# G-U-N/Phased-Consistency-Model

Hardware: NVIDIA H100
Metric: distillation steps/sec (SD1.5 PCM-LoRA, bs=8/GPU) (higher is better)
Workload: dtype bf16

## Files before the change

pcm_b200/csrc/attn.cu:

```cuda
#include <stdio.h>
#include <stdlib.h>
#include "common.cuh"
#include "host_common.h"
#include "../../include/pcm_b200.h"

namespace pcm {

struct AttnParams {
  const bf16 *q, *k, *v, *o, *dout;
  bf16 *out, *dq, *dk, *dv;
  float *lse, *delta;
  int B, H, Sq, Skv, D;
  long long ldq, ldk, ldv, ldo;
  float scale;
};

__device__ __forceinline__ void cp_async16(void* smem_dst, const void* gsrc) {
  asm volatile("cp.async.cg.shared.global [%0], [%1], 16;" ::"r"(smem_u32(smem_dst)), "l"(gsrc)
               : "memory");
}
__device__ __forceinline__ void cp_async_commit() { asm volatile("cp.async.commit_group;" ::: "memory"); }
template <int N>
__device__ __forceinline__ void cp_async_wait() {
  asm volatile("cp.async.wait_group %0;" ::"n"(N) : "memory");
// ... 164 lines not shown
    if (row >= p.Sq) continue;
    const float inv = 1.f / l_run[r];
    bf16* orow = p.out + (static_cast<long long>(b) * p.Sq + row) * p.ldo + h * p.D;
#pragma unroll
    for (int i = 0; i < DP / 8; ++i) {
      const int col = i * 8 + (lane & 3) * 2;
      if (col < p.D)
        *reinterpret_cast<uint32_t*>(orow + col) =
            pack_bf16x2(oacc[i][2 * r] * inv, oacc[i][2 * r + 1] * inv);
    }
    if ((lane & 3) == 0 && p.lse)
      p.lse[(static_cast<long long>(b) * p.H + h) * p.Sq + row] = m_run[r] + log2f(l_run[r]);
  }
}

__global__ void attn_delta_kernel(const AttnParams p) {
  griddep_sync();
  const long long i = blockIdx.x * static_cast<long long>(blockDim.x) + threadIdx.x;
  const long long total = static_cast<long long>(p.B) * p.Sq * p.H;
  if (i >= total) return;
  const int h = static_cast<int>(i % p.H);
  const long long bs = i / p.H;
  const int s = static_cast<int>(bs % p.Sq);
  const int b = static_cast<int>(bs / p.Sq);
  const bf16* o = p.o + bs * p.ldo + h * p.D;
  const bf16* d = p.dout + bs * p.ldo + h * p.D;
  float acc = 0.f;
  for (int c = 0; c < p.D; c += 8) {
    const uint4 u = *reinterpret_cast<const uint4*>(o + c);
    const uint4 w = *reinterpret_cast<const uint4*>(d + c);
    const uint32_t uu[4] = {u.x, u.y, u.z, u.w}, ww[4] = {w.x, w.y, w.z, w.w};
#pragma unroll
    for (int k = 0; k < 4; ++k) {
      const float2 a = unpack_bf16x2(uu[k]), bb = unpack_bf16x2(ww[k]);
      acc += a.x * bb.x + a.y * bb.y;
    }
  }
  p.delta[(static_cast<long long>(b) * p.H + h) * p.Sq + s] = acc;
}

template <int DP>
__global__ void __launch_bounds__(128) attn_bwd_dkdv_kernel(const AttnParams p) {
  griddep_sync();
  constexpr int LDS = DP + 8, BQ = 64, BN = 64, T = 128;
  extern __shared__ __align__(16) uint8_t smem_attn[];
  bf16* sK = reinterpret_cast<bf16*>(smem_attn);
  bf16* sV = sK + BN * LDS;
  bf16* sQ = sV + BN * LDS;
  bf16* sdO = sQ + 2 * BQ * LDS;
  float* sL = reinterpret_cast<float*>(sdO + 2 * BQ * LDS);
  float* sD = sL + 2 * BQ;
  const int tid = threadIdx.x, warp = tid >> 5, lane = tid & 31;
  const int b = blockIdx.z, h = blockIdx.y, n0 = blockIdx.x * BN;
// ... 231 lines not shown
  static bool set = false;
  if (!set) {
    CUDA_TRY(cudaFuncSetAttribute(attn_fwd_kernel<DP>, cudaFuncAttributeMaxDynamicSharedMemorySize,
                                  static_cast<int>(smem)));
    set = true;
  }
  dim3 grid((p.Sq + 127) / 128, p.H, p.B);
  CUDA_TRY(launch_pdl(attn_fwd_kernel<DP>, dim3(grid), dim3(256), smem, stream, p));
  CUDA_TRY(cudaGetLastError());
  return 0;
}

template <int DP>
static int launch_bwd(const AttnParams& p, cudaStream_t stream) {
  constexpr int LDS = DP + 8;
  {
    const long long total = static_cast<long long>(p.B) * p.Sq * p.H;
    CUDA_TRY(launch_pdl(attn_delta_kernel, dim3(static_cast<int>((total + 127) / 128)), dim3(128), 0, stream, p));
  }
  const size_t smem1 = static_cast<size_t>(6 * 64) * LDS * sizeof(bf16) + 4 * 64 * sizeof(float);
  const size_t smem2 = static_cast<size_t>(6 * 64) * LDS * sizeof(bf16);
  static bool set = false;
  if (!set) {
    CUDA_TRY(cudaFuncSetAttribute(attn_bwd_dkdv_kernel<DP>,
                                  cudaFuncAttributeMaxDynamicSharedMemorySize,
                                  static_cast<int>(smem1)));
    CUDA_TRY(cudaFuncSetAttribute(attn_bwd_dq_kernel<DP>,
                                  cudaFuncAttributeMaxDynamicSharedMemorySize,
                                  static_cast<int>(smem2)));
    set = true;
  }
  CUDA_TRY(launch_pdl(attn_bwd_dkdv_kernel<DP>, dim3(dim3((p.Skv + 63) / 64, p.H, p.B)), dim3(128), smem1, stream, p));
  CUDA_TRY(launch_pdl(attn_bwd_dq_kernel<DP>, dim3(dim3((p.Sq + 63) / 64, p.H, p.B)), dim3(128), smem2, stream, p));
  CUDA_TRY(cudaGetLastError());
// ... 111 lines not shown
  AttnParams p{};
  p.q = reinterpret_cast<const bf16*>(q);
  p.k = reinterpret_cast<const bf16*>(k);
  p.v = reinterpret_cast<const bf16*>(v);
  p.o = reinterpret_cast<const bf16*>(o);
  p.dout = reinterpret_cast<const bf16*>(dout);
  p.lse = const_cast<float*>(lse);
  p.delta = delta;
  p.dq = reinterpret_cast<bf16*>(dq);
  p.dk = reinterpret_cast<bf16*>(dk);
  p.dv = reinterpret_cast<bf16*>(dv);
  p.B = B; p.H = H; p.Sq = Sq; p.Skv = Skv; p.D = D;
  p.ldq = ldq; p.ldk = ldk; p.ldv = ldv; p.ldo = ldo;
  p.scale = scale;
  cudaStream_t st = reinterpret_cast<cudaStream_t>(stream);
  if (D <= 64) {
    const long long total = static_cast<long long>(B) * Sq * H;
    CUDA_TRY(launch_pdl(attn_delta_kernel, dim3(static_cast<unsigned>((total + 127) / 128)), dim3(128), 0, st, p));
    const int rc = attn_bwd_wg(q, k, v, dout, lse, delta, dq, dk, dv, B, H, Sq, Skv, D, ldq, ldk, ldv, ldo, scale, st);
    if (rc <= 0) return rc;
  }
  DISPATCH_DP(D, launch_bwd);
}
```

pcm_b200/csrc/attn_wg.cu:

```cuda
#include <type_traits>

#include "common.cuh"
#include "wgmma.cuh"
#include "host_common.h"

namespace pcm {

namespace {

constexpr int kAwThreads = 384;
constexpr int kAwStages = 2;
constexpr int kBwdStages = 3;
constexpr int kTile = 64 * 128;

struct alignas(64) AttnWgParams {
  CUtensorMap q_map, k_map, v_map;
  bf16* out;
  float* lse;
  int H, Sq, Skv, D;
  long long ldo;
  float c;
};

__device__ __forceinline__ void keep_operand(uint32_t (&a)[4][4]) {
// ... 25 lines not shown
    mx[r] = fmaxf(mx[r], __shfl_xor_sync(0xffffffffu, mx[r], 2));
    const float mn = fmaxf(m_run[r], mx[r]);
    alpha[r] = exp2_ftz(m_run[r] - mn);
    m_run[r] = mn;
    rs[r] = 0.f;
  }
#pragma unroll
  for (int i = 0; i < 32; i += 2) {
    const int r = (i >> 1) & 1;
    const float p0 = exp2_ftz(__fsub_rn(s[i], m_run[r])), p1 = exp2_ftz(__fsub_rn(s[i + 1], m_run[r]));
    rs[r] += p0 + p1;
    pa[i >> 3][(i & 7) >> 1] = pack_bf16x2(p0, p1);
  }
}

template <int KB, int NV>
__global__ void __launch_bounds__(kAwThreads, 1) attn_fwd_wg_kernel(const __grid_constant__ AttnWgParams p) {
  static_assert(NV == 64 || (KB == 1 && NV == 40), "trimmed products only for one 64-column block");
  constexpr int KS = (NV + 15) / 16;
  extern __shared__ uint8_t smem_raw[];
  uint8_t* smem = reinterpret_cast<uint8_t*>((reinterpret_cast<uintptr_t>(smem_raw) + 1023) &
                                             ~static_cast<uintptr_t>(1023));
  uint8_t* sQ = smem;
  uint8_t* sK = sQ + 2 * KB * kTile;
  uint8_t* sV = sK + kAwStages * KB * kTile;
  __shared__ __align__(8) uint64_t q_bar;
  __shared__ __align__(8) uint64_t full_bar[kAwStages];
  __shared__ __align__(8) uint64_t empty_bar[kAwStages];

  const int wg = threadIdx.x >> 7;
  const int b = blockIdx.z, h = blockIdx.y, q0 = blockIdx.x * 128;
  const int nblk = (p.Skv + 63) / 64;
  constexpr uint32_t kv_bytes = 2 * KB * kTile;

// ... 33 lines not shown
  const int cw = wg - 1, et = threadIdx.x & 127, warp = et >> 5, lane = et & 31;
  uint8_t* myQ = sQ + cw * KB * kTile;
  mbar_wait(&q_bar, 0);
  if (p.D < KB * 64) {
    const int c0 = p.D >> 3, nch = KB * 8;
    for (int i = et; i < 64 * nch; i += 128) {
      const int row = i / nch, ch = i - row * nch;
      if (ch < c0) continue;
      const uint32_t a = smem_u32(myQ + (ch >> 3) * kTile) + row * 128 + (((ch & 7) ^ (row & 7)) << 4);
      sts128(a, 0u, 0u, 0u, 0u);
    }
    fence_proxy_async();
  }
  asm volatile("bar.sync %0, 128;" ::"r"(1 + cw) : "memory");

  float o[KB][NV / 2];
#pragma unroll
  for (int kb = 0; kb < KB; ++kb)
#pragma unroll
    for (int i = 0; i < NV / 2; ++i) o[kb][i] = 0.f;
  float m_run[2] = {-INFINITY, -INFINITY}, l_run[2] = {0.f, 0.f};
  const uint32_t q_addr = smem_u32(myQ);

  auto block = [&](int j, auto mask) {
    const int st = j % kAwStages;
    mbar_wait(&full_bar[st], (j / kAwStages) & 1);
    const uint32_t k_addr = smem_u32(sK + st * KB * kTile);
    const uint32_t v_addr = smem_u32(sV + st * KB * kTile);
    float s[32];
    wgmma_fence();
#pragma unroll
    for (int kb = 0; kb < KB; ++kb)
#pragma unroll
      for (int k = 0; k < KS; ++k)
        Wgmma<64, 0, 0>::mma(s, wgmma_desc_sw128(q_addr + kb * kTile + k * 32, 16, 1024),
                             wgmma_desc_sw128(k_addr + kb * kTile + k * 32, 16, 1024), (kb | k) != 0 ? 1u : 0u);
    wgmma_commit();
    wgmma_wait<0>();
    wgmma_fence_acc(s);

    float alpha[2], rs[2];
    uint32_t pa[4][4];
    fwd_softmax<decltype(mask)::value>(s, m_run, alpha, rs, pa, p.c, j * 64 + 2 * (lane & 3), p.Skv);
#pragma unroll
    for (int r = 0; r < 2; ++r) l_run[r] = __fmaf_rn(l_run[r], alpha[r], rs[r]);
    if (!__all_sync(0xffffffffu, alpha[0] == 1.f && alpha[1] == 1.f)) {
#pragma unroll
      for (int kb = 0; kb < KB; ++kb)
#pragma unroll
        for (int i = 0; i < NV / 2; ++i) o[kb][i] *= alpha[(i >> 1) & 1];
    }

    wgmma_fence();
#pragma unroll
    for (int kk = 0; kk < 4; ++kk)
#pragma unroll
      for (int kb = 0; kb < KB; ++kb)
        WgmmaRs<NV, 1>::mma(o[kb], pa[kk], wgmma_desc_sw128(v_addr + kb * kTile + kk * 2048, kTile, 1024), 1u);
    wgmma_commit();
    wgmma_wait<0>();
#pragma unroll
    for (int kb = 0; kb < KB; ++kb) wgmma_fence_acc(o[kb]);
    __syncwarp();
    if (et == 0) mbar_arrive(&empty_bar[st]);
  };
  const int nfull = p.Skv / 64;
  for (int j = 0; j < nfull; ++j) block(j, std::false_type());
  if (nfull < nblk) block(nfull, std::true_type());

#pragma unroll
  for (int r = 0; r < 2; ++r) {
    l_run[r] += __shfl_xor_sync(0xffffffffu, l_run[r], 1);
    l_run[r] += __shfl_xor_sync(0xffffffffu, l_run[r], 2);
  }
  const int row0 = q0 + 64 * cw + 16 * warp + (lane >> 2);
#pragma unroll
  for (int r = 0; r < 2; ++r) {
    const int row = row0 + 8 * r;
    if (row >= p.Sq) continue;
    const float inv = 1.f / l_run[r];
    bf16* orow = p.out + (static_cast<long long>(b) * p.Sq + row) * p.ldo + h * p.D;
#pragma unroll
    for (int kb = 0; kb < KB; ++kb)
#pragma unroll
      for (int q = 0; q < NV / 8; ++q) {
        const int col = kb * 64 + 8 * q + 2 * (lane & 3);
        if (col < p.D)
          *reinterpret_cast<uint32_t*>(orow + col) =
              pack_bf16x2(o[kb][4 * q + 2 * r] * inv, o[kb][4 * q + 2 * r + 1] * inv);
      }
    if ((lane & 3) == 0 && p.lse) p.lse[(static_cast<long long>(b) * p.H + h) * p.Sq + row] = m_run[r] + log2f(l_run[r]);
  }
}

struct alignas(64) AttnBwdParams {
  CUtensorMap fix0_map, fix1_map;
  CUtensorMap str0_map, str1_map;
  const float *lse, *delta;
  bf16 *out0, *out1;
  long long ld0, ld1;
  int H, Sq, Skv, D;
  int n_fix, n_str;
  float c, scale;
};

// ... 13 lines not shown
        l = lc[2 * (i >> 2) + e];
        d = dc[2 * (i >> 2) + e];
        ok = rvalid[r];
      } else {
        l = lrow[r];
        d = drow[r];
        ok = !MASK || kcol + 8 * (i >> 2) + e < Skv;
      }
      const float pv = ok ? exp2_ftz(__fmaf_rn(s[i + e], c, -l)) : 0.f;
      s[i + e] = pv;
      dp[i + e] = pv * (dp[i + e] - d);
    }
  }
}

template <bool KV, int NV>
__global__ void __launch_bounds__(kAwThreads, 1) attn_bwd_wg_kernel(const __grid_constant__ AttnBwdParams p) {
  constexpr int kStages = kBwdStages;
  constexpr int KS = (NV + 15) / 16;
  extern __shared__ uint8_t smem_raw[];
  uint8_t* smem = reinterpret_cast<uint8_t*>((reinterpret_cast<uintptr_t>(smem_raw) + 1023) &
                                             ~static_cast<uintptr_t>(1023));
  uint8_t* sF = smem;
  uint8_t* sS = sF + 4 * kTile;
  __shared__ __align__(8) uint64_t f_bar;
  __shared__ __align__(8) uint64_t full_bar[kStages];
  __shared__ __align__(8) uint64_t empty_bar[kStages];
  __shared__ float stats[2][2][2][64];

  const int wg = threadIdx.x >> 7;
  const int b = blockIdx.z, h = blockIdx.y, r0 = blockIdx.x * 128;
  const int nblk = (p.n_str + 63) / 64;
  const int col0 = h * p.D;

  if (threadIdx.x == 0) {
    tma_prefetch_desc(&p.fix0_map);
    tma_prefetch_desc(&p.fix1_map);
    tma_prefetch_desc(&p.str0_map);
    tma_prefetch_desc(&p.str1_map);
    mbar_init(&f_bar, 1);
    for (int i = 0; i < kStages; ++i) {
      mbar_init(&full_bar[i], 1);
      mbar_init(&empty_bar[i], 2);
    }
    fence_barrier_init();
  }
  __syncthreads();
  griddep_sync();

  if (wg == 0) {
    regs_dealloc<40>();
    if (threadIdx.x == 0) {
      mbar_arrive_expect_tx(&f_bar, 4 * kTile);
      for (int w = 0; w < 2; ++w) {
        tma_load_3d(sF + (2 * w) * kTile, &p.fix0_map, &f_bar, col0, r0 + 64 * w, b);
        tma_load_3d(sF + (2 * w + 1) * kTile, &p.fix1_map, &f_bar, col0, r0 + 64 * w, b);
      }
      for (int j = 0; j < nblk; ++j) {
        const int st = j % kStages;
        mbar_wait(&empty_bar[st], ((j / kStages) & 1) ^ 1);
        mbar_arrive_expect_tx(&full_bar[st], 2 * kTile);
        tma_load_3d(sS + (2 * st) * kTile, &p.str0_map, &full_bar[st], col0, j * 64, b);
        tma_load_3d(sS + (2 * st + 1) * kTile, &p.str1_map, &full_bar[st], col0, j * 64, b);
      }
    }
    return;
  }

  regs_alloc<232>();
  const int cw = wg - 1, et = threadIdx.x & 127, warp = et >> 5, lane = et & 31;
  uint8_t* myF = sF + 2 * cw * kTile;
  mbar_wait(&f_bar, 0);
  if (p.D < 64) {
    const int c0 = p.D >> 3;
    for (int i = et; i < 2 * 64 * 8; i += 128) {
      const int t = i >> 9, row = (i >> 3) & 63, ch = i & 7;
      if (ch < c0) continue;
      sts128(smem_u32(myF + t * kTile) + row * 128 + ((ch ^ (row & 7)) << 4), 0u, 0u, 0u, 0u);
    }
    fence_proxy_async();
  }
  asm volatile("bar.sync %0, 128;" ::"r"(1 + cw) : "memory");

  const float* L = p.lse + (static_cast<long long>(b) * p.H + h) * p.Sq;
  const float* Dl = p.delta + (static_cast<long long>(b) * p.H + h) * p.Sq;
  const int frow = r0 + 64 * cw + 16 * warp + (lane >> 2);
  float lrow[2] = {0.f, 0.f}, drow[2] = {0.f, 0.f};
  bool rvalid[2];
#pragma unroll
  for (int r = 0; r < 2; ++r) {
    rvalid[r] = frow + 8 * r < p.n_fix;
    if (!KV) {
      lrow[r] = rvalid[r] ? L[frow + 8 * r] : INFINITY;
      drow[r] = rvalid[r] ? Dl[frow + 8 * r] : 0.f;
    }
  }
  float acc0[NV / 2], acc1[NV / 2];
#pragma unroll
  for (int i = 0; i < NV / 2; ++i) acc0[i] = acc1[i] = 0.f;
  const uint32_t f0 = smem_u32(myF), f1 = f0 + kTile;
  const bool ragged = !KV && (p.Skv & 63) != 0;
  float s[32], dp[32];
  uint32_t pa[4][4], dsa[4][4];

  auto issue_sdp = [&](int st) {
    const uint32_t s0 = smem_u32(sS + 2 * st * kTile), s1 = s0 + kTile;
    Wgmma<64, 0, 0>::mma_first(s, wgmma_desc_sw128(f0, 16, 1024), wgmma_desc_sw128(s0, 16, 1024));
    Wgmma<64, 0, 0>::mma_first(dp, wgmma_desc_sw128(f1, 16, 1024), wgmma_desc_sw128(s1, 16, 1024));
#pragma unroll
    for (int k = 1; k < KS; ++k) {
      Wgmma<64, 0, 0>::mma(s, wgmma_desc_sw128(f0 + k * 32, 16, 1024), wgmma_desc_sw128(s0 + k * 32, 16, 1024), 1u);
      Wgmma<64, 0, 0>::mma(dp, wgmma_desc_sw128(f1 + k * 32, 16, 1024), wgmma_desc_sw128(s1 + k * 32, 16, 1024), 1u);
    }
    wgmma_commit();
  };
  auto issue_acc = [&](int st) {
    const uint32_t s0 = smem_u32(sS + 2 * st * kTile), s1 = s0 + kTile;
#pragma unroll
    for (int kk = 0; kk < 4; ++kk) {
      WgmmaRs<NV, 1>::mma(acc0, dsa[kk], wgmma_desc_sw128(s0 + kk * 2048, kTile, 1024), 1u);
      if (KV) WgmmaRs<NV, 1>::mma(acc1, pa[kk], wgmma_desc_sw128(s1 + kk * 2048, kTile, 1024), 1u);
    }
    wgmma_commit();
  };
  auto load_stat = [&](int j) {
    const int qi = j * 64 + (et & 63);
    if (et < 64) return qi < p.Sq ? L[qi] : INFINITY;
    return qi < p.Sq ? Dl[qi] : 0.f;
  };
  auto publish_stat = [&](int j, float v) {
    stats[cw][j & 1][et >> 6][et & 63] = v;
    asm volatile("bar.sync %0, 128;" ::"r"(1 + cw) : "memory");
  };
  auto elementwise = [&](int j) {
    const int kcol = j * 64 + 2 * (lane & 3);
    float lc[16], dc[16];
// ... 28 lines not shown
  pack_operand(dsa, dp);

  for (int j = 1; j < nblk; ++j) {
    const int st = j % kStages, pst = (j - 1) % kStages;
    mbar_wait(&full_bar[st], (j / kStages) & 1);
    wgmma_fence();
    issue_sdp(st);
    issue_acc(pst);
    if (KV) nxt = load_stat(j + 1);
    wgmma_wait<1>();
    wgmma_fence_acc(s);
    wgmma_fence_acc(dp);
    elementwise(j);
    if (KV) publish_stat(j + 1, nxt);
    wgmma_wait<0>();
    wgmma_fence_acc(acc0);
    wgmma_fence_acc(acc1);
    keep_operand(pa);
    keep_operand(dsa);
    __syncwarp();
    if (et == 0) mbar_arrive(&empty_bar[pst]);
    pack_operand(pa, s);
    pack_operand(dsa, dp);
  }
  wgmma_fence();
  issue_acc((nblk - 1) % kStages);
  wgmma_wait<0>();
  wgmma_fence_acc(acc0);
  wgmma_fence_acc(acc1);
  keep_operand(pa);
  keep_operand(dsa);

#pragma unroll
  for (int r = 0; r < 2; ++r) {
    if (!rvalid[r]) continue;
    const long long row = static_cast<long long>(b) * p.n_fix + frow + 8 * r;
    bf16* o0 = p.out0 + row * p.ld0 + col0;
    bf16* o1 = KV ? p.out1 + row * p.ld1 + col0 : nullptr;
#pragma unroll
    for (int q = 0; q < NV / 8; ++q) {
      const int col = 8 * q + 2 * (lane & 3);
      if (col < p.D) {
        *reinterpret_cast<uint32_t*>(o0 + col) =
            pack_bf16x2(acc0[4 * q + 2 * r] * p.scale, acc0[4 * q + 2 * r + 1] * p.scale);
        if (KV) *reinterpret_cast<uint32_t*>(o1 + col) = pack_bf16x2(acc1[4 * q + 2 * r], acc1[4 * q + 2 * r + 1]);
      }
    }
  }
}

int encode_seq_map(CUtensorMap* m, const void* base, int HD, int S, int B, long long ld) {
  if ((reinterpret_cast<uintptr_t>(base) & 15) != 0 || (ld & 7) != 0)
    return set_error("attention: tensor map base not 16-byte aligned or row stride not a multiple of 8");
  cuuint64_t dims[3] = {static_cast<cuuint64_t>(HD), static_cast<cuuint64_t>(S), static_cast<cuuint64_t>(B)};
  cuuint64_t strides[2] = {static_cast<cuuint64_t>(ld) * 2, static_cast<cuuint64_t>(ld) * 2 * S};
  cuuint32_t box[3] = {64, 64, 1}, estr[3] = {1, 1, 1};
  return encode_tmap(m, base, 3, dims, strides, box, estr);
}

template <int KB, int NV>
cudaError_t launch_fwd(dim3 grid, cudaStream_t stream, const AttnWgParams& p) {
  const size_t smem = KB * (2 + 2 * kAwStages) * kTile + 1024;
  static bool attr = false;
  if (!attr) {
    const cudaError_t e = cudaFuncSetAttribute(attn_fwd_wg_kernel<KB, NV>, cudaFuncAttributeMaxDynamicSharedMemorySize,
                                               static_cast<int>(smem));
    if (e != cudaSuccess) return e;
    attr = true;
  }
  return launch_pdl(attn_fwd_wg_kernel<KB, NV>, grid, dim3(kAwThreads), smem, stream, p);
}

template <bool KV, int NV>
cudaError_t launch_bwd(dim3 grid, cudaStream_t stream, const AttnBwdParams& p) {
  const size_t smem = (4 + 2 * kBwdStages) * kTile + 1024;
  static bool attr = false;
  if (!attr) {
    const cudaError_t e = cudaFuncSetAttribute(attn_bwd_wg_kernel<KV, NV>, cudaFuncAttributeMaxDynamicSharedMemorySize,
                                               static_cast<int>(smem));
    if (e != cudaSuccess) return e;
    attr = true;
  }
  return launch_pdl(attn_bwd_wg_kernel<KV, NV>, grid, dim3(kAwThreads), smem, stream, p);
}

}

int attn_fwd_wg(const void* q, const void* k, const void* v, void* out, float* lse, int B, int H, int Sq,
                int Skv, int D, long long ldq, long long ldk, long long ldv, long long ldo, float scale,
                cudaStream_t stream) {
  if (D % 8 != 0 || D > 128) return 1;
  static AttnWgParams p;
  memset(&p, 0, sizeof(p));
  int rc;
  if ((rc = encode_seq_map(&p.q_map, q, H * D, Sq, B, ldq)) != 0) return rc;
  if ((rc = encode_seq_map(&p.k_map, k, H * D, Skv, B, ldk)) != 0) return rc;
  if ((rc = encode_seq_map(&p.v_map, v, H * D, Skv, B, ldv)) != 0) return rc;
  p.out = reinterpret_cast<bf16*>(out);
  p.lse = lse;
  p.H = H; p.Sq = Sq; p.Skv = Skv; p.D = D; p.ldo = ldo;
  p.c = scale * 1.4426950408889634f;
  const dim3 grid((Sq + 127) / 128, H, B);
  if (D <= 40)
    CUDA_TRY((launch_fwd<1, 40>)(grid, stream, p));
  else if (D <= 64)
    CUDA_TRY((launch_fwd<1, 64>)(grid, stream, p));
  else
    CUDA_TRY((launch_fwd<2, 64>)(grid, stream, p));
  CUDA_TRY(cudaGetLastError());
  return 0;
}

int attn_bwd_wg(const void* q, const void* k, const void* v, const void* dout, const float* lse,
                const float* delta, void* dq, void* dk, void* dv, int B, int H, int Sq, int Skv, int D,
                long long ldq, long long ldk, long long ldv, long long ldo, float scale, cudaStream_t stream) {
  if (D % 8 != 0 || D > 64) return 1;
  static AttnBwdParams pk, pq;
  memset(&pk, 0, sizeof(pk));
  int rc;
  if ((rc = encode_seq_map(&pk.fix0_map, k, H * D, Skv, B, ldk)) != 0) return rc;
  if ((rc = encode_seq_map(&pk.fix1_map, v, H * D, Skv, B, ldv)) != 0) return rc;
  if ((rc = encode_seq_map(&pk.str0_map, q, H * D, Sq, B, ldq)) != 0) return rc;
  if ((rc = encode_seq_map(&pk.str1_map, dout, H * D, Sq, B, ldo)) != 0) return rc;
  pk.lse = lse; pk.delta = delta;
  pk.H = H; pk.Sq = Sq; pk.Skv = Skv; pk.D = D;
  pk.c = scale * 1.4426950408889634f;
  pq = pk;
  pk.out0 = reinterpret_cast<bf16*>(dk); pk.ld0 = ldk;
  pk.out1 = reinterpret_cast<bf16*>(dv); pk.ld1 = ldv;
  pk.n_fix = Skv; pk.n_str = Sq; pk.scale = scale;
  pq.fix0_map = pk.str0_map; pq.fix1_map = pk.str1_map;
  pq.str0_map = pk.fix0_map; pq.str1_map = pk.fix1_map;
  pq.out0 = reinterpret_cast<bf16*>(dq); pq.ld0 = ldq;
  pq.out1 = nullptr; pq.ld1 = 0;
  pq.n_fix = Sq; pq.n_str = Skv; pq.scale = scale;
  const dim3 gk((Skv + 127) / 128, H, B), gq((Sq + 127) / 128, H, B);
  if (D <= 40) {
    CUDA_TRY((launch_bwd<true, 40>)(gk, stream, pk));
    CUDA_TRY((launch_bwd<false, 40>)(gq, stream, pq));
  } else {
    CUDA_TRY((launch_bwd<true, 64>)(gk, stream, pk));
    CUDA_TRY((launch_bwd<false, 64>)(gq, stream, pq));
  }
  CUDA_TRY(cudaGetLastError());
  return 0;
}

}
```

pcm_b200/csrc/wgmma.cuh:

```cuda
#pragma once
#include <stdint.h>

namespace pcm {

template <int N, int TA, int TB>
struct Wgmma;

template <int TA, int TB>
struct Wgmma<32, TA, TB> {
  __device__ __forceinline__ static void mma(float (&d)[16], uint64_t a, uint64_t b, uint32_t acc) {
    asm volatile(
        "{\n\t.reg .pred p;\n\t"
        "setp.ne.b32 p, %18, 0;\n\t"
        "wgmma.mma_async.sync.aligned.m64n32k16.f32.bf16.bf16 "
        "{%0, %1, %2, %3, %4, %5, %6, %7, %8, %9, %10, %11, %12, %13, %14, %15}, "
        "%16, %17, p, 1, 1, %19, %20;\n\t}"
        : "+f"(d[0]), "+f"(d[1]), "+f"(d[2]), "+f"(d[3]), "+f"(d[4]), "+f"(d[5]), "+f"(d[6]), "+f"(d[7]), "+f"(d[8]), "+f"(d[9]), "+f"(d[10]), "+f"(d[11]), "+f"(d[12]), "+f"(d[13]), "+f"(d[14]), "+f"(d[15])
        : "l"(a), "l"(b), "r"(acc), "n"(TA), "n"(TB));
  }
};

template <int TA, int TB>
struct Wgmma<64, TA, TB> {
  __device__ __forceinline__ static void mma(float (&d)[32], uint64_t a, uint64_t b, uint32_t acc) {
// ... 92 lines not shown
    asm volatile(
        "{\n\t.reg .pred p;\n\t"
        "setp.ne.b32 p, %130, 0;\n\t"
        "wgmma.mma_async.sync.aligned.m64n256k16.f32.bf16.bf16 "
        "{%0, %1, %2, %3, %4, %5, %6, %7, %8, %9, %10, %11, %12, %13, %14, %15, %16, %17, %18, %19, %20, %21, %22, %23, %24, %25, %26, %27, %28, %29, %30, %31, %32, %33, %34, %35, %36, %37, %38, %39, %40, %41, %42, %43, %44, %45, %46, %47, %48, %49, %50, %51, %52, %53, %54, %55, %56, %57, %58, %59, %60, %61, %62, %63, %64, %65, %66, %67, %68, %69, %70, %71, %72, %73, %74, %75, %76, %77, %78, %79, %80, %81, %82, %83, %84, %85, %86, %87, %88, %89, %90, %91, %92, %93, %94, %95, %96, %97, %98, %99, %100, %101, %102, %103, %104, %105, %106, %107, %108, %109, %110, %111, %112, %113, %114, %115, %116, %117, %118, %119, %120, %121, %122, %123, %124, %125, %126, %127}, "
        "%128, %129, p, 1, 1, %131, %132;\n\t}"
        : "+f"(d[0]), "+f"(d[1]), "+f"(d[2]), "+f"(d[3]), "+f"(d[4]), "+f"(d[5]), "+f"(d[6]), "+f"(d[7]), "+f"(d[8]), "+f"(d[9]), "+f"(d[10]), "+f"(d[11]), "+f"(d[12]), "+f"(d[13]), "+f"(d[14]), "+f"(d[15]), "+f"(d[16]), "+f"(d[17]), "+f"(d[18]), "+f"(d[19]), "+f"(d[20]), "+f"(d[21]), "+f"(d[22]), "+f"(d[23]), "+f"(d[24]), "+f"(d[25]), "+f"(d[26]), "+f"(d[27]), "+f"(d[28]), "+f"(d[29]), "+f"(d[30]), "+f"(d[31]), "+f"(d[32]), "+f"(d[33]), "+f"(d[34]), "+f"(d[35]), "+f"(d[36]), "+f"(d[37]), "+f"(d[38]), "+f"(d[39]), "+f"(d[40]), "+f"(d[41]), "+f"(d[42]), "+f"(d[43]), "+f"(d[44]), "+f"(d[45]), "+f"(d[46]), "+f"(d[47]), "+f"(d[48]), "+f"(d[49]), "+f"(d[50]), "+f"(d[51]), "+f"(d[52]), "+f"(d[53]), "+f"(d[54]), "+f"(d[55]), "+f"(d[56]), "+f"(d[57]), "+f"(d[58]), "+f"(d[59]), "+f"(d[60]), "+f"(d[61]), "+f"(d[62]), "+f"(d[63]), "+f"(d[64]), "+f"(d[65]), "+f"(d[66]), "+f"(d[67]), "+f"(d[68]), "+f"(d[69]), "+f"(d[70]), "+f"(d[71]), "+f"(d[72]), "+f"(d[73]), "+f"(d[74]), "+f"(d[75]), "+f"(d[76]), "+f"(d[77]), "+f"(d[78]), "+f"(d[79]), "+f"(d[80]), "+f"(d[81]), "+f"(d[82]), "+f"(d[83]), "+f"(d[84]), "+f"(d[85]), "+f"(d[86]), "+f"(d[87]), "+f"(d[88]), "+f"(d[89]), "+f"(d[90]), "+f"(d[91]), "+f"(d[92]), "+f"(d[93]), "+f"(d[94]), "+f"(d[95]), "+f"(d[96]), "+f"(d[97]), "+f"(d[98]), "+f"(d[99]), "+f"(d[100]), "+f"(d[101]), "+f"(d[102]), "+f"(d[103]), "+f"(d[104]), "+f"(d[105]), "+f"(d[106]), "+f"(d[107]), "+f"(d[108]), "+f"(d[109]), "+f"(d[110]), "+f"(d[111]), "+f"(d[112]), "+f"(d[113]), "+f"(d[114]), "+f"(d[115]), "+f"(d[116]), "+f"(d[117]), "+f"(d[118]), "+f"(d[119]), "+f"(d[120]), "+f"(d[121]), "+f"(d[122]), "+f"(d[123]), "+f"(d[124]), "+f"(d[125]), "+f"(d[126]), "+f"(d[127])
        : "l"(a), "l"(b), "r"(acc), "n"(TA), "n"(TB));
  }
};

template <int N, int TB>
struct WgmmaRs;

template <int TB>
struct WgmmaRs<40, TB> {
  __device__ __forceinline__ static void mma(float (&d)[20], const uint32_t (&a)[4], uint64_t b, uint32_t acc) {
    asm volatile(
        "{\n\t.reg .pred p;\n\t"
        "setp.ne.b32 p, %25, 0;\n\t"
        "wgmma.mma_async.sync.aligned.m64n40k16.f32.bf16.bf16 "
        "{%0, %1, %2, %3, %4, %5, %6, %7, %8, %9, %10, %11, %12, %13, %14, %15, %16, %17, %18, %19}, "
        "{%20, %21, %22, %23}, %24, p, 1, 1, %26;\n\t}"
        : "+f"(d[0]), "+f"(d[1]), "+f"(d[2]), "+f"(d[3]), "+f"(d[4]), "+f"(d[5]), "+f"(d[6]), "+f"(d[7]), "+f"(d[8]), "+f"(d[9]), "+f"(d[10]), "+f"(d[11]), "+f"(d[12]), "+f"(d[13]), "+f"(d[14]), "+f"(d[15]), "+f"(d[16]), "+f"(d[17]), "+f"(d[18]), "+f"(d[19])
        : "r"(a[0]), "r"(a[1]), "r"(a[2]), "r"(a[3]), "l"(b), "r"(acc), "n"(TB));
  }
};

template <int TB>
struct WgmmaRs<64, TB> {
// ... 14 lines not shown
```

Baseline: 9.080.

## Extend wgmma attention to head dims 80 and 160 with trimmed tail tiles

Generalizes the wgmma forward and backward attention kernels to several 64-column head blocks plus a narrow trailing tile (n16/n32/n40/n64), so head dims 80 and 160 use the TMA/wgmma path instead of padded tiles or the older kernel. The backward wgmma path now also covers D=80. The delta kernel is rewritten to stage o and dout rows through shared memory with coalesced loads. This adds register pressure (a 232-register cap for the backward accumulators) and more template instantiations.

```diff
diff --git a/pcm_b200/csrc/attn.cu b/pcm_b200/csrc/attn.cu
--- a/pcm_b200/csrc/attn.cu
+++ b/pcm_b200/csrc/attn.cu
@@ -202,21 +202,35 @@
   }
 }
 
-__global__ void attn_delta_kernel(const AttnParams p) {
+constexpr int kDeltaRows = 128;
+
+static size_t attn_delta_smem(int D) {
+  return 2 * static_cast<size_t>(kDeltaRows) * ((D >> 3) | 1) * sizeof(uint4);
+}
+
+__global__ void __launch_bounds__(kDeltaRows) attn_delta_kernel(const AttnParams p) {
+  extern __shared__ uint4 sdelta[];
   griddep_sync();
-  const long long i = blockIdx.x * static_cast<long long>(blockDim.x) + threadIdx.x;
-  const long long total = static_cast<long long>(p.B) * p.Sq * p.H;
-  if (i >= total) return;
-  const int h = static_cast<int>(i % p.H);
-  const long long bs = i / p.H;
-  const int s = static_cast<int>(bs % p.Sq);
-  const int b = static_cast<int>(bs / p.Sq);
-  const bf16* o = p.o + bs * p.ldo + h * p.D;
-  const bf16* d = p.dout + bs * p.ldo + h * p.D;
+  const int total = p.B * p.Sq * p.H;
+  const int i0 = blockIdx.x * kDeltaRows;
+  const int rows = min(kDeltaRows, total - i0);
+  const int nc = p.D >> 3, ns = nc | 1;
+  uint4* so = sdelta;
+  uint4* sd = sdelta + kDeltaRows * ns;
+#pragma unroll 4
+  for (int j = threadIdx.x; j < rows * nc; j += kDeltaRows) {
+    const int r = j / nc, c = j - r * nc, i = i0 + r;
+    const int bs = i / p.H, h = i - bs * p.H;
+    const long long off = static_cast<long long>(bs) * p.ldo + h * p.D + 8 * c;
+    so[r * ns + c] = *reinterpret_cast<const uint4*>(p.o + off);
+    sd[r * ns + c] = *reinterpret_cast<const uint4*>(p.dout + off);
+  }
+  __syncthreads();
+  const int r = threadIdx.x;
+  if (r >= rows) return;
   float acc = 0.f;
-  for (int c = 0; c < p.D; c += 8) {
-    const uint4 u = *reinterpret_cast<const uint4*>(o + c);
-    const uint4 w = *reinterpret_cast<const uint4*>(d + c);
+  for (int c = 0; c < nc; ++c) {
+    const uint4 u = so[r * ns + c], w = sd[r * ns + c];
     const uint32_t uu[4] = {u.x, u.y, u.z, u.w}, ww[4] = {w.x, w.y, w.z, w.w};
 #pragma unroll
     for (int k = 0; k < 4; ++k) {
@@ -224,7 +238,22 @@
       acc += a.x * bb.x + a.y * bb.y;
     }
   }
+  const int i = i0 + r, bs = i / p.H, h = i - bs * p.H;
+  const int s = bs % p.Sq, b = bs / p.Sq;
   p.delta[(static_cast<long long>(b) * p.H + h) * p.Sq + s] = acc;
+}
+
+static int launch_delta(const AttnParams& p, cudaStream_t stream) {
+  static bool set = false;
+  if (!set) {
+    CUDA_TRY(cudaFuncSetAttribute(attn_delta_kernel, cudaFuncAttributeMaxDynamicSharedMemorySize,
+                                  static_cast<int>(attn_delta_smem(160))));
+    set = true;
+  }
+  const int total = p.B * p.Sq * p.H;
+  CUDA_TRY(launch_pdl(attn_delta_kernel, dim3((total + kDeltaRows - 1) / kDeltaRows), dim3(kDeltaRows),
+                      attn_delta_smem(p.D), stream, p));
+  return 0;
 }
 
 template <int DP>
@@ -486,10 +515,7 @@
 template <int DP>
 static int launch_bwd(const AttnParams& p, cudaStream_t stream) {
   constexpr int LDS = DP + 8;
-  {
-    const long long total = static_cast<long long>(p.B) * p.Sq * p.H;
-    CUDA_TRY(launch_pdl(attn_delta_kernel, dim3(static_cast<int>((total + 127) / 128)), dim3(128), 0, stream, p));
-  }
+  if (const int rc = launch_delta(p, stream)) return rc;
   const size_t smem1 = static_cast<size_t>(6 * 64) * LDS * sizeof(bf16) + 4 * 64 * sizeof(float);
   const size_t smem2 = static_cast<size_t>(6 * 64) * LDS * sizeof(bf16);
   static bool set = false;
@@ -631,9 +657,8 @@
   p.ldq = ldq; p.ldk = ldk; p.ldv = ldv; p.ldo = ldo;
   p.scale = scale;
   cudaStream_t st = reinterpret_cast<cudaStream_t>(stream);
-  if (D <= 64) {
-    const long long total = static_cast<long long>(B) * Sq * H;
-    CUDA_TRY(launch_pdl(attn_delta_kernel, dim3(static_cast<unsigned>((total + 127) / 128)), dim3(128), 0, st, p));
+  if (D <= 80) {
+    if (const int rc = launch_delta(p, st)) return rc;
     const int rc = attn_bwd_wg(q, k, v, dout, lse, delta, dq, dk, dv, B, H, Sq, Skv, D, ldq, ldk, ldv, ldo, scale, st);
     if (rc <= 0) return rc;
   }
diff --git a/pcm_b200/csrc/attn_wg.cu b/pcm_b200/csrc/attn_wg.cu
--- a/pcm_b200/csrc/attn_wg.cu
+++ b/pcm_b200/csrc/attn_wg.cu
@@ -63,10 +63,11 @@
   }
 }
 
-template <int KB, int NV>
+template <int KB, int NT>
 __global__ void __launch_bounds__(kAwThreads, 1) attn_fwd_wg_kernel(const __grid_constant__ AttnWgParams p) {
-  static_assert(NV == 64 || (KB == 1 && NV == 40), "trimmed products only for one 64-column block");
-  constexpr int KS = (NV + 15) / 16;
+  static_assert(NT == 16 || NT == 32 || NT == 40 || NT == 64, "no register-A wgmma of this width");
+  constexpr int KF = KB - 1;
+  constexpr int KS = (NT + 15) / 16;
   extern __shared__ uint8_t smem_raw[];
   uint8_t* smem = reinterpret_cast<uint8_t*>((reinterpret_cast<uintptr_t>(smem_raw) + 1023) &
                                              ~static_cast<uintptr_t>(1023));
@@ -130,11 +131,13 @@
   }
   asm volatile("bar.sync %0, 128;" ::"r"(1 + cw) : "memory");
 
-  float o[KB][NV / 2];
-#pragma unroll
-  for (int kb = 0; kb < KB; ++kb)
-#pragma unroll
-    for (int i = 0; i < NV / 2; ++i) o[kb][i] = 0.f;
+  float of[KF > 0 ? KF : 1][32], ot[NT / 2];
+#pragma unroll
+  for (int kb = 0; kb < KF; ++kb)
+#pragma unroll
+    for (int i = 0; i < 32; ++i) of[kb][i] = 0.f;
+#pragma unroll
+  for (int i = 0; i < NT / 2; ++i) ot[i] = 0.f;
   float m_run[2] = {-INFINITY, -INFINITY}, l_run[2] = {0.f, 0.f};
   const uint32_t q_addr = smem_u32(myQ);
 
@@ -148,7 +151,7 @@
 #pragma unroll
     for (int kb = 0; kb < KB; ++kb)
 #pragma unroll
-      for (int k = 0; k < KS; ++k)
+      for (int k = 0; k < (kb < KF ? 4 : KS); ++k)
         Wgmma<64, 0, 0>::mma(s, wgmma_desc_sw128(q_addr + kb * kTile + k * 32, 16, 1024),
                              wgmma_desc_sw128(k_addr + kb * kTile + k * 32, 16, 1024), (kb | k) != 0 ? 1u : 0u);
     wgmma_commit();
@@ -162,21 +165,26 @@
     for (int r = 0; r < 2; ++r) l_run[r] = __fmaf_rn(l_run[r], alpha[r], rs[r]);
     if (!__all_sync(0xffffffffu, alpha[0] == 1.f && alpha[1] == 1.f)) {
 #pragma unroll
-      for (int kb = 0; kb < KB; ++kb)
-#pragma unroll
-        for (int i = 0; i < NV / 2; ++i) o[kb][i] *= alpha[(i >> 1) & 1];
+      for (int kb = 0; kb < KF; ++kb)
+#pragma unroll
+        for (int i = 0; i < 32; ++i) of[kb][i] *= alpha[(i >> 1) & 1];
+#pragma unroll
+      for (int i = 0; i < NT / 2; ++i) ot[i] *= alpha[(i >> 1) & 1];
     }
 
     wgmma_fence();
 #pragma unroll
-    for (int kk = 0; kk < 4; ++kk)
-#pragma unroll
-      for (int kb = 0; kb < KB; ++kb)
-        WgmmaRs<NV, 1>::mma(o[kb], pa[kk], wgmma_desc_sw128(v_addr + kb * kTile + kk * 2048, kTile, 1024), 1u);
+    for (int kk = 0; kk < 4; ++kk) {
+#pragma unroll
+      for (int kb = 0; kb < KF; ++kb)
+        WgmmaRs<64, 1>::mma(of[kb], pa[kk], wgmma_desc_sw128(v_addr + kb * kTile + kk * 2048, kTile, 1024), 1u);
+      WgmmaRs<NT, 1>::mma(ot, pa[kk], wgmma_desc_sw128(v_addr + KF * kTile + kk * 2048, kTile, 1024), 1u);
+    }
     wgmma_commit();
     wgmma_wait<0>();
 #pragma unroll
-    for (int kb = 0; kb < KB; ++kb) wgmma_fence_acc(o[kb]);
+    for (int kb = 0; kb < KF; ++kb) wgmma_fence_acc(of[kb]);
+    wgmma_fence_acc(ot);
     __syncwarp();
     if (et == 0) mbar_arrive(&empty_bar[st]);
   };
@@ -197,14 +205,18 @@
     const float inv = 1.f / l_run[r];
     bf16* orow = p.out + (static_cast<long long>(b) * p.Sq + row) * p.ldo + h * p.D;
 #pragma unroll
-    for (int kb = 0; kb < KB; ++kb)
-#pragma unroll
-      for (int q = 0; q < NV / 8; ++q) {
+    for (int kb = 0; kb < KF; ++kb)
+#pragma unroll
+      for (int q = 0; q < 8; ++q) {
         const int col = kb * 64 + 8 * q + 2 * (lane & 3);
-        if (col < p.D)
-          *reinterpret_cast<uint32_t*>(orow + col) =
-              pack_bf16x2(o[kb][4 * q + 2 * r] * inv, o[kb][4 * q + 2 * r + 1] * inv);
-      }
+        *reinterpret_cast<uint32_t*>(orow + col) = pack_bf16x2(of[kb][4 * q + 2 * r] * inv, of[kb][4 * q + 2 * r + 1] * inv);
+      }
+#pragma unroll
+    for (int q = 0; q < NT / 8; ++q) {
+      const int col = KF * 64 + 8 * q + 2 * (lane & 3);
+      if (col < p.D)
+        *reinterpret_cast<uint32_t*>(orow + col) = pack_bf16x2(ot[4 * q + 2 * r] * inv, ot[4 * q + 2 * r + 1] * inv);
+    }
     if ((lane & 3) == 0 && p.lse) p.lse[(static_cast<long long>(b) * p.H + h) * p.Sq + row] = m_run[r] + log2f(l_run[r]);
   }
 }
@@ -248,15 +260,17 @@
   }
 }
 
-template <bool KV, int NV>
+template <bool KV, int KB, int NT>
 __global__ void __launch_bounds__(kAwThreads, 1) attn_bwd_wg_kernel(const __grid_constant__ AttnBwdParams p) {
+  static_assert((KB == 1 && (NT == 40 || NT == 64)) || (KB == 2 && NT == 16), "accumulators must fit in 232 registers");
   constexpr int kStages = kBwdStages;
-  constexpr int KS = (NV + 15) / 16;
+  constexpr int KF = KB - 1;
+  constexpr int KS = (NT + 15) / 16;
   extern __shared__ uint8_t smem_raw[];
   uint8_t* smem = reinterpret_cast<uint8_t*>((reinterpret_cast<uintptr_t>(smem_raw) + 1023) &
                                              ~static_cast<uintptr_t>(1023));
   uint8_t* sF = smem;
-  uint8_t* sS = sF + 4 * kTile;
+  uint8_t* sS = sF + 4 * KB * kTile;
   __shared__ __align__(8) uint64_t f_bar;
   __shared__ __align__(8) uint64_t full_bar[kStages];
   __shared__ __align__(8) uint64_t empty_bar[kStages];
@@ -285,17 +299,20 @@
   if (wg == 0) {
     regs_dealloc<40>();
     if (threadIdx.x == 0) {
-      mbar_arrive_expect_tx(&f_bar, 4 * kTile);
-      for (int w = 0; w < 2; ++w) {
-        tma_load_3d(sF + (2 * w) * kTile, &p.fix0_map, &f_bar, col0, r0 + 64 * w, b);
-        tma_load_3d(sF + (2 * w + 1) * kTile, &p.fix1_map, &f_bar, col0, r0 + 64 * w, b);
-      }
+      mbar_arrive_expect_tx(&f_bar, 4 * KB * kTile);
+      for (int w = 0; w < 2; ++w)
+        for (int kb = 0; kb < KB; ++kb) {
+          tma_load_3d(sF + (2 * w * KB + kb) * kTile, &p.fix0_map, &f_bar, col0 + kb * 64, r0 + 64 * w, b);
+          tma_load_3d(sF + ((2 * w + 1) * KB + kb) * kTile, &p.fix1_map, &f_bar, col0 + kb * 64, r0 + 64 * w, b);
+        }
       for (int j = 0; j < nblk; ++j) {
         const int st = j % kStages;
         mbar_wait(&empty_bar[st], ((j / kStages) & 1) ^ 1);
-        mbar_arrive_expect_tx(&full_bar[st], 2 * kTile);
-        tma_load_3d(sS + (2 * st) * kTile, &p.str0_map, &full_bar[st], col0, j * 64, b);
-        tma_load_3d(sS + (2 * st + 1) * kTile, &p.str1_map, &full_bar[st], col0, j * 64, b);
+        mbar_arrive_expect_tx(&full_bar[st], 2 * KB * kTile);
+        for (int kb = 0; kb < KB; ++kb) {
+          tma_load_3d(sS + (2 * st * KB + kb) * kTile, &p.str0_map, &full_bar[st], col0 + kb * 64, j * 64, b);
+          tma_load_3d(sS + ((2 * st + 1) * KB + kb) * kTile, &p.str1_map, &full_bar[st], col0 + kb * 64, j * 64, b);
+        }
       }
     }
     return;
@@ -303,14 +320,15 @@
 
   regs_alloc<232>();
   const int cw = wg - 1, et = threadIdx.x & 127, warp = et >> 5, lane = et & 31;
-  uint8_t* myF = sF + 2 * cw * kTile;
+  uint8_t* myF = sF + 2 * cw * KB * kTile;
   mbar_wait(&f_bar, 0);
-  if (p.D < 64) {
+  if (p.D < KB * 64) {
+    constexpr int kChLog = KB == 1 ? 3 : 4;
     const int c0 = p.D >> 3;
-    for (int i = et; i < 2 * 64 * 8; i += 128) {
-      const int t = i >> 9, row = (i >> 3) & 63, ch = i & 7;
+    for (int i = et; i < 2 * 64 * 8 * KB; i += 128) {
+      const int t = i >> (6 + kChLog), row = (i >> kChLog) & 63, ch = i & (8 * KB - 1);
       if (ch < c0) continue;
-      sts128(smem_u32(myF + t * kTile) + row * 128 + ((ch ^ (row & 7)) << 4), 0u, 0u, 0u, 0u);
+      sts128(smem_u32(myF + (t * KB + (ch >> 3)) * kTile) + row * 128 + (((ch & 7) ^ (row & 7)) << 4), 0u, 0u, 0u, 0u);
     }
     fence_proxy_async();
   }
@@ -329,31 +347,55 @@
       drow[r] = rvalid[r] ? Dl[frow + 8 * r] : 0.f;
     }
   }
-  float acc0[NV / 2], acc1[NV / 2];
-#pragma unroll
-  for (int i = 0; i < NV / 2; ++i) acc0[i] = acc1[i] = 0.f;
-  const uint32_t f0 = smem_u32(myF), f1 = f0 + kTile;
+  float acc0f[KF > 0 ? KF : 1][32], acc1f[KF > 0 ? KF : 1][32], acc0t[NT / 2], acc1t[NT / 2];
+#pragma unroll
+  for (int kb = 0; kb < KF; ++kb)
+#pragma unroll
+    for (int i = 0; i < 32; ++i) acc0f[kb][i] = acc1f[kb][i] = 0.f;
+#pragma unroll
+  for (int i = 0; i < NT / 2; ++i) acc0t[i] = acc1t[i] = 0.f;
+  auto fence_accs = [&]() {
+#pragma unroll
+    for (int kb = 0; kb < KF; ++kb) {
+      wgmma_fence_acc(acc0f[kb]);
+      wgmma_fence_acc(acc1f[kb]);
+    }
+    wgmma_fence_acc(acc0t);
+    wgmma_fence_acc(acc1t);
+  };
+  const uint32_t f0 = smem_u32(myF), f1 = f0 + KB * kTile;
   const bool ragged = !KV && (p.Skv & 63) != 0;
   float s[32], dp[32];
   uint32_t pa[4][4], dsa[4][4];
 
   auto issue_sdp = [&](int st) {
-    const uint32_t s0 = smem_u32(sS + 2 * st * kTile), s1 = s0 + kTile;
+    const uint32_t s0 = smem_u32(sS + 2 * st * KB * kTile), s1 = s0 + KB * kTile;
     Wgmma<64, 0, 0>::mma_first(s, wgmma_desc_sw128(f0, 16, 1024), wgmma_desc_sw128(s0, 16, 1024));
     Wgmma<64, 0, 0>::mma_first(dp, wgmma_desc_sw128(f1, 16, 1024), wgmma_desc_sw128(s1, 16, 1024));
 #pragma unroll
-    for (int k = 1; k < KS; ++k) {
-      Wgmma<64, 0, 0>::mma(s, wgmma_desc_sw128(f0 + k * 32, 16, 1024), wgmma_desc_sw128(s0 + k * 32, 16, 1024), 1u);
-      Wgmma<64, 0, 0>::mma(dp, wgmma_desc_sw128(f1 + k * 32, 16, 1024), wgmma_desc_sw128(s1 + k * 32, 16, 1024), 1u);
-    }
+    for (int kb = 0; kb < KB; ++kb)
+#pragma unroll
+      for (int k = kb == 0 ? 1 : 0; k < (kb < KF ? 4 : KS); ++k) {
+        const int o = kb * kTile + k * 32;
+        Wgmma<64, 0, 0>::mma(s, wgmma_desc_sw128(f0 + o, 16, 1024), wgmma_desc_sw128(s0 + o, 16, 1024), 1u);
+        Wgmma<64, 0, 0>::mma(dp, wgmma_desc_sw128(f1 + o, 16, 1024), wgmma_desc_sw128(s1 + o, 16, 1024), 1u);
+      }
     wgmma_commit();
   };
   auto issue_acc = [&](int st) {
-    const uint32_t s0 = smem_u32(sS + 2 * st * kTile), s1 = s0 + kTile;
+    const uint32_t s0 = smem_u32(sS + 2 * st * KB * kTile), s1 = s0 + KB * kTile;
 #pragma unroll
     for (int kk = 0; kk < 4; ++kk) {
-      WgmmaRs<NV, 1>::mma(acc0, dsa[kk], wgmma_desc_sw128(s0 + kk * 2048, kTile, 1024), 1u);
-      if (KV) WgmmaRs<NV, 1>::mma(acc1, pa[kk], wgmma_desc_sw128(s1 + kk * 2048, kTile, 1024), 1u);
+#pragma unroll
+      for (int kb = 0; kb < KF; ++kb)
+        WgmmaRs<64, 1>::mma(acc0f[kb], dsa[kk], wgmma_desc_sw128(s0 + kb * kTile + kk * 2048, kTile, 1024), 1u);
+      WgmmaRs<NT, 1>::mma(acc0t, dsa[kk], wgmma_desc_sw128(s0 + KF * kTile + kk * 2048, kTile, 1024), 1u);
+      if (KV) {
+#pragma unroll
+        for (int kb = 0; kb < KF; ++kb)
+          WgmmaRs<64, 1>::mma(acc1f[kb], pa[kk], wgmma_desc_sw128(s1 + kb * kTile + kk * 2048, kTile, 1024), 1u);
+        WgmmaRs<NT, 1>::mma(acc1t, pa[kk], wgmma_desc_sw128(s1 + KF * kTile + kk * 2048, kTile, 1024), 1u);
+      }
     }
     wgmma_commit();
   };
@@ -412,8 +454,7 @@
     elementwise(j);
     if (KV) publish_stat(j + 1, nxt);
     wgmma_wait<0>();
-    wgmma_fence_acc(acc0);
-    wgmma_fence_acc(acc1);
+    fence_accs();
     keep_operand(pa);
     keep_operand(dsa);
     __syncwarp();
@@ -424,8 +465,7 @@
   wgmma_fence();
   issue_acc((nblk - 1) % kStages);
   wgmma_wait<0>();
-  wgmma_fence_acc(acc0);
-  wgmma_fence_acc(acc1);
+  fence_accs();
   keep_operand(pa);
   keep_operand(dsa);
 
@@ -436,12 +476,22 @@
     bf16* o0 = p.out0 + row * p.ld0 + col0;
     bf16* o1 = KV ? p.out1 + row * p.ld1 + col0 : nullptr;
 #pragma unroll
-    for (int q = 0; q < NV / 8; ++q) {
-      const int col = 8 * q + 2 * (lane & 3);
+    for (int kb = 0; kb < KF; ++kb)
+#pragma unroll
+      for (int q = 0; q < 8; ++q) {
+        const int col = kb * 64 + 8 * q + 2 * (lane & 3);
+        *reinterpret_cast<uint32_t*>(o0 + col) =
+            pack_bf16x2(acc0f[kb][4 * q + 2 * r] * p.scale, acc0f[kb][4 * q + 2 * r + 1] * p.scale);
+        if (KV)
+          *reinterpret_cast<uint32_t*>(o1 + col) = pack_bf16x2(acc1f[kb][4 * q + 2 * r], acc1f[kb][4 * q + 2 * r + 1]);
+      }
+#pragma unroll
+    for (int q = 0; q < NT / 8; ++q) {
+      const int col = KF * 64 + 8 * q + 2 * (lane & 3);
       if (col < p.D) {
         *reinterpret_cast<uint32_t*>(o0 + col) =
-            pack_bf16x2(acc0[4 * q + 2 * r] * p.scale, acc0[4 * q + 2 * r + 1] * p.scale);
-        if (KV) *reinterpret_cast<uint32_t*>(o1 + col) = pack_bf16x2(acc1[4 * q + 2 * r], acc1[4 * q + 2 * r + 1]);
+            pack_bf16x2(acc0t[4 * q + 2 * r] * p.scale, acc0t[4 * q + 2 * r + 1] * p.scale);
+        if (KV) *reinterpret_cast<uint32_t*>(o1 + col) = pack_bf16x2(acc1t[4 * q + 2 * r], acc1t[4 * q + 2 * r + 1]);
       }
     }
   }
@@ -456,30 +506,30 @@
   return encode_tmap(m, base, 3, dims, strides, box, estr);
 }
 
-template <int KB, int NV>
+template <int KB, int NT>
 cudaError_t launch_fwd(dim3 grid, cudaStream_t stream, const AttnWgParams& p) {
   const size_t smem = KB * (2 + 2 * kAwStages) * kTile + 1024;
   static bool attr = false;
   if (!attr) {
-    const cudaError_t e = cudaFuncSetAttribute(attn_fwd_wg_kernel<KB, NV>, cudaFuncAttributeMaxDynamicSharedMemorySize,
+    const cudaError_t e = cudaFuncSetAttribute(attn_fwd_wg_kernel<KB, NT>, cudaFuncAttributeMaxDynamicSharedMemorySize,
                                                static_cast<int>(smem));
     if (e != cudaSuccess) return e;
     attr = true;
   }
-  return launch_pdl(attn_fwd_wg_kernel<KB, NV>, grid, dim3(kAwThreads), smem, stream, p);
-}
-
-template <bool KV, int NV>
+  return launch_pdl(attn_fwd_wg_kernel<KB, NT>, grid, dim3(kAwThreads), smem, stream, p);
+}
+
+template <bool KV, int KB, int NT>
 cudaError_t launch_bwd(dim3 grid, cudaStream_t stream, const AttnBwdParams& p) {
-  const size_t smem = (4 + 2 * kBwdStages) * kTile + 1024;
+  const size_t smem = KB * (4 + 2 * kBwdStages) * kTile + 1024;
   static bool attr = false;
   if (!attr) {
-    const cudaError_t e = cudaFuncSetAttribute(attn_bwd_wg_kernel<KV, NV>, cudaFuncAttributeMaxDynamicSharedMemorySize,
-                                               static_cast<int>(smem));
+    const cudaError_t e = cudaFuncSetAttribute(attn_bwd_wg_kernel<KV, KB, NT>,
+                                               cudaFuncAttributeMaxDynamicSharedMemorySize, static_cast<int>(smem));
     if (e != cudaSuccess) return e;
     attr = true;
   }
-  return launch_pdl(attn_bwd_wg_kernel<KV, NV>, grid, dim3(kAwThreads), smem, stream, p);
+  return launch_pdl(attn_bwd_wg_kernel<KV, KB, NT>, grid, dim3(kAwThreads), smem, stream, p);
 }
 
 }
@@ -487,7 +537,7 @@
 int attn_fwd_wg(const void* q, const void* k, const void* v, void* out, float* lse, int B, int H, int Sq,
                 int Skv, int D, long long ldq, long long ldk, long long ldv, long long ldo, float scale,
                 cudaStream_t stream) {
-  if (D % 8 != 0 || D > 128) return 1;
+  if (D % 8 != 0 || D > 192) return 1;
   static AttnWgParams p;
   memset(&p, 0, sizeof(p));
   int rc;
@@ -503,8 +553,16 @@
     CUDA_TRY((launch_fwd<1, 40>)(grid, stream, p));
   else if (D <= 64)
     CUDA_TRY((launch_fwd<1, 64>)(grid, stream, p));
+  else if (D <= 80)
+    CUDA_TRY((launch_fwd<2, 16>)(grid, stream, p));
+  else if (D <= 96)
+    CUDA_TRY((launch_fwd<2, 32>)(grid, stream, p));
+  else if (D <= 128)
+    CUDA_TRY((launch_fwd<2, 64>)(grid, stream, p));
+  else if (D <= 160)
+    CUDA_TRY((launch_fwd<3, 32>)(grid, stream, p));
   else
-    CUDA_TRY((launch_fwd<2, 64>)(grid, stream, p));
+    CUDA_TRY((launch_fwd<3, 64>)(grid, stream, p));
   CUDA_TRY(cudaGetLastError());
   return 0;
 }
@@ -512,7 +570,7 @@
 int attn_bwd_wg(const void* q, const void* k, const void* v, const void* dout, const float* lse,
                 const float* delta, void* dq, void* dk, void* dv, int B, int H, int Sq, int Skv, int D,
                 long long ldq, long long ldk, long long ldv, long long ldo, float scale, cudaStream_t stream) {
-  if (D % 8 != 0 || D > 64) return 1;
+  if (D % 8 != 0 || D > 80) return 1;
   static AttnBwdParams pk, pq;
   memset(&pk, 0, sizeof(pk));
   int rc;
@@ -534,11 +592,14 @@
   pq.n_fix = Sq; pq.n_str = Skv; pq.scale = scale;
   const dim3 gk((Skv + 127) / 128, H, B), gq((Sq + 127) / 128, H, B);
   if (D <= 40) {
-    CUDA_TRY((launch_bwd<true, 40>)(gk, stream, pk));
-    CUDA_TRY((launch_bwd<false, 40>)(gq, stream, pq));
+    CUDA_TRY((launch_bwd<true, 1, 40>)(gk, stream, pk));
+    CUDA_TRY((launch_bwd<false, 1, 40>)(gq, stream, pq));
+  } else if (D <= 64) {
+    CUDA_TRY((launch_bwd<true, 1, 64>)(gk, stream, pk));
+    CUDA_TRY((launch_bwd<false, 1, 64>)(gq, stream, pq));
   } else {
-    CUDA_TRY((launch_bwd<true, 64>)(gk, stream, pk));
-    CUDA_TRY((launch_bwd<false, 64>)(gq, stream, pq));
+    CUDA_TRY((launch_bwd<true, 2, 16>)(gk, stream, pk));
+    CUDA_TRY((launch_bwd<false, 2, 16>)(gq, stream, pq));
   }
   CUDA_TRY(cudaGetLastError());
   return 0;
diff --git a/pcm_b200/csrc/wgmma.cuh b/pcm_b200/csrc/wgmma.cuh
--- a/pcm_b200/csrc/wgmma.cuh
+++ b/pcm_b200/csrc/wgmma.cuh
@@ -130,6 +130,34 @@
 struct WgmmaRs;
 
 template <int TB>
+struct WgmmaRs<16, TB> {
+  __device__ __forceinline__ static void mma(float (&d)[8], const uint32_t (&a)[4], uint64_t b, uint32_t acc) {
+    asm volatile(
+        "{\n\t.reg .pred p;\n\t"
+        "setp.ne.b32 p, %13, 0;\n\t"
+        "wgmma.mma_async.sync.aligned.m64n16k16.f32.bf16.bf16 "
+        "{%0, %1, %2, %3, %4, %5, %6, %7}, "
+        "{%8, %9, %10, %11}, %12, p, 1, 1, %14;\n\t}"
+        : "+f"(d[0]), "+f"(d[1]), "+f"(d[2]), "+f"(d[3]), "+f"(d[4]), "+f"(d[5]), "+f"(d[6]), "+f"(d[7])
+        : "r"(a[0]), "r"(a[1]), "r"(a[2]), "r"(a[3]), "l"(b), "r"(acc), "n"(TB));
+  }
+};
+
+template <int TB>
+struct WgmmaRs<32, TB> {
+  __device__ __forceinline__ static void mma(float (&d)[16], const uint32_t (&a)[4], uint64_t b, uint32_t acc) {
+    asm volatile(
+        "{\n\t.reg .pred p;\n\t"
+        "setp.ne.b32 p, %21, 0;\n\t"
+        "wgmma.mma_async.sync.aligned.m64n32k16.f32.bf16.bf16 "
+        "{%0, %1, %2, %3, %4, %5, %6, %7, %8, %9, %10, %11, %12, %13, %14, %15}, "
+        "{%16, %17, %18, %19}, %20, p, 1, 1, %22;\n\t}"
+        : "+f"(d[0]), "+f"(d[1]), "+f"(d[2]), "+f"(d[3]), "+f"(d[4]), "+f"(d[5]), "+f"(d[6]), "+f"(d[7]), "+f"(d[8]), "+f"(d[9]), "+f"(d[10]), "+f"(d[11]), "+f"(d[12]), "+f"(d[13]), "+f"(d[14]), "+f"(d[15])
+        : "r"(a[0]), "r"(a[1]), "r"(a[2]), "r"(a[3]), "l"(b), "r"(acc), "n"(TB));
+  }
+};
+
+template <int TB>
 struct WgmmaRs<40, TB> {
   __device__ __forceinline__ static void mma(float (&d)[20], const uint32_t (&a)[4], uint64_t b, uint32_t acc) {
     asm volatile(
```

Result: faster. 9.239, median of 6 (+1.8%).
